# mic-rud/Learned-Compression-of-Point-Cloud-Geometry-and-Attributes

Hardware: AMD Instinct MI355X
Metric: encode+decode Mpoints/sec (higher is better)
Workload: dtype f32

## Files before the change

### include/pcc_hip.h

```cpp
#ifndef PCC_HIP_H
#define PCC_HIP_H

#include <stdint.h>

#ifdef __cplusplus
extern "C" {
#endif

#define PCC_OK 0
#define PCC_ERR_ARG (-1)
#define PCC_ERR_HIP (-2)
#define PCC_ERR_UNSUPPORTED (-3)
#define PCC_ERR_DATA (-4)

#define PCC_ACT_NONE 0
#define PCC_ACT_RELU 1
#define PCC_ACT_LEAKY_RELU 2

int pcc_version(void);
const char* pcc_last_error(void);
int pcc_device_count(void);
int pcc_device_name(int dev, char* out, int out_len);

int64_t pcc_hash_capacity(int64_t n);
// ... 30 lines not shown
int pcc_voxelize(const float* xyz, const int32_t* batch, int64_t n, int32_t nbatch, const float* attr, int32_t c,
                 float origin_x, float origin_y, float origin_z, float voxel, int32_t rounding, uint64_t* keys,
                 int32_t* vals, int64_t cap, int32_t* scratch, int32_t* out_coords, int32_t* out_first,
                 int32_t* out_npts, int64_t* out_sum, int32_t* out_row, int64_t* out_count, void* stream);

int pcc_kernel_map(const int32_t* out_coords, int64_t n_out, const uint64_t* in_keys,
                   const int32_t* in_vals, int64_t in_cap, int32_t ksize, int32_t step,
                   int32_t sign, int32_t* nbr, uint32_t* row_mask, int64_t* pair_count,
                   void* stream);

int pcc_pair_count(const uint32_t* row_mask, int64_t n_out, int64_t* pair_count, void* stream);

int64_t pcc_order_scratch_bytes(int64_t n);
int pcc_order_rows_by_mask(const uint32_t* row_mask, const int32_t* coords, int64_t n,
                           int32_t block_log2, int32_t tensor_stride, int32_t* order, uint32_t* group_mask32,
                           void* scratch, int64_t scratch_bytes, void* stream);
int pcc_permute_map_rows(const int32_t* nbr, const int32_t* order, int64_t n, int32_t K, int32_t* nbr_sorted, void* stream);

int64_t pcc_small_map_max(void);
int32_t pcc_small_paths(int32_t mask);
int pcc_small_kernel_map(const int32_t* out_coords, int64_t n_out, const uint64_t* in_keys, const int32_t* in_vals, int64_t in_cap,
                         int32_t ksize, int32_t step, int32_t sign, int32_t* nbr, uint32_t* row_mask, int32_t* order,
                         uint32_t* group_mask32, void* scratch, int64_t scratch_bytes, void* stream);

int64_t pcc_conv_packed_elems(int32_t K, int32_t cin, int32_t cout);
int pcc_conv_pack_weights(const float* w, int32_t K, int32_t cin, int32_t cout, float* w_packed,
                          void* stream);
int pcc_conv_fwd(const float* fin, int64_t n_in, int32_t cin, const float* w, const float* w_packed,
                 const float* bias, const int32_t* nbr, const int32_t* order,
                 const uint32_t* group_mask32, int32_t K, float* fout, int64_t n_out, int32_t cout,
                 int32_t act, const float* film, const float* residual, void* stream);

int64_t pcc_conv_small_max(int64_t workgroups);

int pcc_conv_kernel_name(int32_t mode, int64_t n_in, int32_t cin, int32_t cout, int64_t n_out, int32_t K, int32_t has_nbr,
                         char* buf, int32_t len);

int64_t pcc_conv_packed_elems_bf16(int32_t K, int32_t cin, int32_t cout);
int pcc_conv_pack_weights_bf16(const float* w, int32_t K, int32_t cin, int32_t cout, uint16_t* w_packed, void* stream);
int pcc_conv_fwd_bf16(const uint16_t* fin, int64_t n_in, int32_t cin, const uint16_t* w_packed, const float* bias,
                      const int32_t* nbr, const int32_t* order, const uint32_t* group_mask32, int32_t K, float* fout,
                      int64_t n_out, int32_t cout, int32_t act, const float* film, const float* residual, void* stream);

int pcc_epilogue_fwd(const float* c, const float* film, const float* residual, int64_t n, int32_t channels, int32_t act,
                     float* out, void* stream);
int pcc_epilogue_bwd(const float* dout, const float* c, const float* film, int64_t n, int32_t channels, int32_t act,
                     float* dc, float* dfilm, void* stream);

int64_t pcc_cast_colsum_scratch_elems(int32_t channels);
int pcc_cast_colsum(const float* x, int64_t n, int32_t channels, uint16_t* out_bf16, float* colsum, float* scratch,
                    int64_t scratch_elems, void* stream);

int64_t pcc_conv_packed_elems_x3(int32_t K, int32_t cin, int32_t cout);
int pcc_conv_pack_weights_x3(const float* w, int32_t K, int32_t cin, int32_t cout, uint16_t* w_packed, void* stream);
int pcc_conv_fwd_x3(const float* fin, int64_t n_in, int32_t cin, const uint16_t* w_packed, const float* bias,
                    const int32_t* nbr, const int32_t* order, const uint32_t* group_mask32, int32_t K, float* fout,
                    int64_t n_out, int32_t cout, int32_t act, const float* film, const float* residual, void* stream);

int pcc_im2col_thin(const float* fin, int32_t cin, const int32_t* nbr, int64_t n_out, int32_t K, float* out, int32_t k2,
                    void* stream);

int pcc_gather_sum_fwd(const float* scores, int32_t ld, const int32_t* nbr, int32_t K, int32_t cout,
                       const float* bias, float* out, int64_t n_out, int32_t act, void* stream);

int pcc_gather_rows(const float* src, int32_t c, const int32_t* idx, int64_t n, float* out,
                    int32_t accumulate, void* stream);
// ... 126 lines not shown
```

### learned-compression-of-point-cloud-geometry-and-attributes_amd/_build.py

```python
import os
import subprocess

_HERE = os.path.dirname(os.path.abspath(__file__))
SO_PATH = os.path.join(_HERE, "libpcc_hip.so")

NO_SCRATCH = {
    "conv": ("conv_small_kernel", "conv_mfma_buf_kernel", "conv_mfma_kernel"),
    "rans_lanes": ("rans_lanes_encode_kernel", "rans_lanes_pack_kernel", "rans_lanes_decode_kernel"),
    "chconv": ("chconv_kernel",),
    "augment": ("jitter_partial_kernel", "jitter_mean_kernel", "jitter_apply_kernel", "first_rows_clear_kernel",
                "first_rows_insert_kernel", "first_rows_flag_kernel", "first_rows_finalize_kernel"),
    "normals": ("estimate_normals_kernel",),
    "voxelize": ("first_rows_clear_kernel", "first_rows_insert_kernel", "first_rows_flag_kernel", "first_rows_finalize_kernel",
                 "voxelize_accumulate_kernel"),
    "raht": ("raht_plan_kernel", "raht_step_kernel", "raht_fold_kernel"),
}


def build(force=False):
    args = ["make", "-s", "-C", os.path.join(_HERE, "csrc"), "-j4"]
    if force:
        subprocess.check_call(args + ["clean"])
    subprocess.check_call(args)
    for stem, kernels in NO_SCRATCH.items():
        check_kernel_resources(os.path.join(_HERE, "build", stem + ".resources.txt"), kernels)
    check_small_kernel_lds_reads()
    return SO_PATH


def check_small_kernel_lds_reads(obj=None):
    import glob
    import shutil
    objdump = "/opt/rocm/lib/llvm/bin/llvm-objdump"
    obj = obj or os.path.join(_HERE, "build", "conv.o")
    if not os.path.exists(objdump) or not os.path.exists(obj):
        raise RuntimeError(f"cannot lint conv_small_kernel: {objdump} or {obj} is missing")
    tmp = os.path.join(_HERE, "build", "_lint")
    shutil.rmtree(tmp, ignore_errors=True)
    os.makedirs(tmp)
    local = os.path.join(tmp, "conv.o")
# ... 84 lines not shown
```

### learned-compression-of-point-cloud-geometry-and-attributes_amd/csrc/conv.hip

```cpp
#include <stdlib.h>

#include <type_traits>

#include "common.h"

namespace pcc {

typedef float f32x2 __attribute__((ext_vector_type(2)));
typedef float f32x4 __attribute__((ext_vector_type(4)));
typedef __bf16 bf16x8 __attribute__((ext_vector_type(8)));

struct ConvArgs {
    const float* fin;
    const float* w;
    const float* wp;
    const float* bias;
    const int32_t* nbr;
    const int32_t* order;
    const uint32_t* gmask;
    float* fout;
    const float* film;
    const float* residual;
    int64_t n_in, n_out;
    int cin, cout, coutp, K, act;
// ... 172 lines not shown
__device__ __forceinline__ unsigned live_tiles(const uint32_t (&mmask)[MT], int k) {
    unsigned live = 0;
#pragma unroll
    for (int m = 0; m < MT; ++m) live |= ((mmask[m] >> k) & 1u) << m;
    return live;
}

template <int MT, class F>
__device__ __forceinline__ void for_live_pattern(unsigned live, F&& block) {
    if constexpr (MT == 1) {
        if (live) block(std::integral_constant<unsigned, 1u>{});
    } else {
        static_assert(MT == 2, "live-pattern dispatch written for MT <= 2");
        if (live == 3u) block(std::integral_constant<unsigned, 3u>{});
        else if (live == 1u) block(std::integral_constant<unsigned, 1u>{});
        else if (live == 2u) block(std::integral_constant<unsigned, 2u>{});
    }
}

template <int MT, int NT>
__device__ __forceinline__ void conv_store_tiles(const ConvArgs& a, const f32x16 (&acc)[MT][NT], int64_t pos0, int col0, int h) {
#pragma unroll
    for (int m = 0; m < MT; ++m) {
#pragma unroll
        for (int n = 0; n < NT; ++n) {
            const int col = col0 + 32 * n;
            if (col >= a.cout) continue;
            const float bcol = conv_bias(a, col);
#pragma unroll
            for (int reg = 0; reg < 16; ++reg) {
                const int64_t pos = pos0 + 32 * m + 4 * h + mfma32_row(reg);
                if (pos >= a.n_out) continue;
                conv_store(a, a.order ? a.order[pos] : pos, col, acc[m][n][reg], bcol);
            }
        }
    }
}

template <int BM, int BN, int WAVES_M, int WAVES_N, bool HAS_NBR>
__global__ __launch_bounds__(256) void conv_mfma_kernel(const ConvArgs a) {
    constexpr int RPT = BM / 32;
    constexpr int WM = BM / WAVES_M, WN = BN / WAVES_N;
    constexpr int MT = WM / 32, NT = WN / 32;
    constexpr int A_LD = A_LD_DMA;
    constexpr int A_ELEMS = BM * A_LD;
    constexpr int W_ELEMS = 8 * BN * 4;
    constexpr int W_LOADS = (8 * BN) / 256;
    static_assert(WAVES_M * WAVES_N == 4 && MT >= 1 && NT >= 1 && W_LOADS >= 1, "bad tiling");

    extern __shared__ __attribute__((aligned(16))) float smem[];
    float* As = smem;
    float* Ws = smem + 2 * A_ELEMS;

    const int t = threadIdx.x;
    const int lane = t & 63, wid = t >> 6;
    const int r = lane & 31, h = lane >> 5;
    const int wrow = (wid / WAVES_N) * WM, wcol = (wid % WAVES_N) * WN;

    const int ntiles_n = a.coutp / BN;
    const int64_t tile = blockIdx.x / ntiles_n;
    const int nt = blockIdx.x - (int)(tile * ntiles_n);
    const int64_t row0 = tile * BM;
    const int CCH = a.cin / 32;
    const int K = a.K;

    uint32_t mmask[MT];
// ... 310 lines not shown
                if constexpr (c + 1 < CCH) {
                    dma(k, std::integral_constant<int, c + 1>{}, std::integral_constant<int, buf ^ 1>{});
                } else {
                    set_src(knext >= 0);
                    dma(knext >= 0 ? knext : k, std::integral_constant<int, 0>{}, std::integral_constant<int, buf ^ 1>{});
                    load_idx(kn2);
                }
                compute(std::integral_constant<int, buf>{}, live);
                __syncthreads();
            });
            const bool more = knext >= 0;
            k = more ? knext : k;
            rem = rem2;
            return more;
        };

        load_idx(k);
        set_src(true);
        dma(k, std::integral_constant<int, 0>{}, std::integral_constant<int, 0>{});
        load_idx(rem ? __builtin_ctz(rem) : k);
        __syncthreads();
        while (true) {
            if (!offset_body(std::integral_constant<int, 0>{})) break;
            if constexpr (CCH & 1) {
                if (!offset_body(std::integral_constant<int, 1>{})) break;
            }
        }
    }

    conv_store_tiles(a, acc, row0 + wrow, nt * BN + wcol + r, h);
#endif
}

template <int SC, int NS>
constexpr int conv_small_lds_bytes() { return (NS * SC * (32 * 32 + 8 * 32 * 4) + 32 * 32) * (int)sizeof(float); }

template <int SC, int NS>
__global__ __launch_bounds__(512) void conv_small_kernel(const ConvArgs a) {
#if defined(__HIP_DEVICE_COMPILE__)
    constexpr int A_STAGE = SC * 32 * 32;
    constexpr int W_STAGE = SC * 8 * 32 * 4;
    constexpr int STAGE = A_STAGE + W_STAGE;
    constexpr int DMAS = 2 * SC;
    static_assert(NS >= 2 && (NS - 1) * DMAS <= 63, "vmcnt is a 6-bit counter");
    extern __shared__ __attribute__((aligned(16))) float smem[];
    int* idx_s = reinterpret_cast<int*>(smem + NS * STAGE);

    const int t = threadIdx.x;
    const int lane = t & 63;
    const int wave_u = __builtin_amdgcn_readfirstlane(t >> 6);
    const int K = a.K;
    const int ntiles_n = a.coutp / 32;
    const int64_t tile = blockIdx.x / ntiles_n;
    const int nt = blockIdx.x - (int)(tile * ntiles_n);
    const int64_t row0 = tile * 32;
    uint32_t tmask = (K >= 32) ? 0xffffffffu : ((1u << K) - 1u);
    if (a.gmask) tmask &= a.gmask[row0 >> 5];
    tmask = __builtin_amdgcn_readfirstlane(tmask);
    const int CG = (a.cin / 32) / SC;
    const int total = __builtin_popcount(tmask) * CG;
    constexpr int WAIT_FIRST = (NS - 1) * DMAS, WAIT_LOOP = (NS - 2) * DMAS;

    if (tmask != 0u) {
        for (int e = t; e < 32 * K; e += 512) {
            const int lr = e / K;
            const int64_t pos = row0 + lr;
// ... 237 lines not shown
            for (int64_t u = w; u < words; ++u) idx_s[u] = src[u];
        }
    }
    __syncthreads();
    if ((int64_t)threadIdx.x >= rows) return;
    const int32_t* mine = idx_s + threadIdx.x * 27;
    float acc[COUT];
#pragma unroll
    for (int c = 0; c < COUT; ++c) acc[c] = 0.0f;
#pragma unroll
    for (int k0 = 0; k0 < 27; k0 += 9) {
        int idx[9];
        float v[9][COUT];
#pragma unroll
        for (int u = 0; u < 9; ++u) idx[u] = mine[k0 + u];
#pragma unroll
        for (int u = 0; u < 9; ++u) {
            const float* sp = scores + (int64_t)(idx[u] >= 0 ? idx[u] : 0) * ld + (k0 + u) * COUT;
#pragma unroll
            for (int c = 0; c < COUT; ++c) v[u][c] = sp[c];
        }
#pragma unroll
        for (int u = 0; u < 9; ++u)
            if (idx[u] >= 0) {
#pragma unroll
                for (int c = 0; c < COUT; ++c) acc[c] += v[u][c];
            }
    }
    float* o = out + (row0 + threadIdx.x) * COUT;
#pragma unroll
    for (int c = 0; c < COUT; ++c) o[c] = apply_act(acc[c] + (bias ? bias[c] : 0.0f), act);
}

enum ConvMode { CONV_F32 = 0, CONV_BF16 = 1, CONV_X3 = 2 };
static const char* const CONV_ENTRY[] = {"pcc_conv_fwd", "pcc_conv_fwd_bf16", "pcc_conv_fwd_x3"};
static const char* const CONV_TAG[] = {"", "[bf16]", "[x3]"};

enum ConvFamily { FAM_THIN, FAM_SMALL, FAM_BUF, FAM_GLOBAL };

struct ConvPlan {
    ConvFamily family;
    int bm, bn, wm, wn;
    int cch;
    int sc, ns;
    int cpt;
};

constexpr int64_t FILL_WGS = 768;
constexpr int64_t ROW32_MAX_WGS = 3000;

static inline int round_up32(int v) { return (v + 31) / 32 * 32; }

static bool fits_buffer_path(const ConvArgs& a) {
    const uint64_t lim = BUF_OOB;
    return (uint64_t)a.n_in * a.cin * 4 <= lim && (uint64_t)a.n_out * a.K * 4 <= lim && (uint64_t)a.K * a.cin * a.coutp * 4 <= lim;
}

static int conv_path() {
    static int path = -1;
    if (path < 0) { const char* e = getenv("PCC_CONV_PATH"); path = (e && e[0] == 'g') ? 1 : 0; }
    return path;
}

static int64_t g_small_max = -1;
static int64_t small_max_value() {
    if (g_small_max < 0) { const char* e = getenv("PCC_CONV_SMALL_MAX"); g_small_max = e ? atoll(e) : 640; }
    return g_small_max;
}

static bool thin_cin(int cin) {
    for (int c : {1, 2, 3, 4, 6, 8, 12, 16, 24})
        if (cin == c) return true;
    return false;
}

static int check_shape(const ConvArgs& a, ConvMode mode, const char* who) {
    PCC_REQUIRE(a.K >= 1 && a.K <= 27, "%s: K=%d out of range", who, a.K);
    if (mode == CONV_F32) PCC_REQUIRE(a.cin % 32 != 0 || a.cin <= 256, "%s: MFMA path supports cin <= 256 (got %d)", who, a.cin);
    if (mode == CONV_BF16) PCC_REQUIRE(a.cin % 64 == 0 && a.cin <= 256, "%s: cin must be a multiple of 64 up to 256 (got %d)", who, a.cin);
    if (mode == CONV_X3) PCC_REQUIRE(a.cin % 32 == 0 && a.cin <= 256, "%s: cin must be a multiple of 32 up to 256 (got %d)", who, a.cin);
    PCC_REQUIRE(a.nbr != nullptr || (a.K == 1 && a.n_in == a.n_out), "%s: nbr == NULL needs K == 1 and n_in == n_out", who);
    return PCC_OK;
}

static int plan_conv(const ConvArgs& a, ConvMode mode, ConvPlan& p, const char* who) {
    p = ConvPlan{};
    if (mode == CONV_F32 && a.cin % 32 != 0) {
        if (!thin_cin(a.cin)) {
            pcc::set_error("%s: unsupported cin=%d (need a multiple of 32 or one of 1,2,3,4,6,8,12,16,24)", who, a.cin);
            return PCC_ERR_UNSUPPORTED;
        }
        const size_t lds = (size_t)a.K * a.cin * a.cout * sizeof(float);
        PCC_REQUIRE(lds <= 160 * 1024, "conv(thin): weights %zu B exceed the 160 KB of LDS (cin=%d cout=%d K=%d)", lds, a.cin, a.cout, a.K);
        p.family = FAM_THIN;
        p.cpt = (a.cout % 8 == 0) ? 8 : (a.cout % 4 == 0) ? 4 : (a.cout % 2 == 0) ? 2 : 1;
        return PCC_OK;
    }
    const bool wide = a.coutp % 128 == 0;
    p.family = FAM_BUF;
    p.cch = a.cin / (mode == CONV_BF16 ? 64 : 32);
    if (mode == CONV_F32) {
        const bool buffer = conv_path() == 0 && fits_buffer_path(a);
        const int64_t wgs32 = ((a.n_out + 31) / 32) * (a.coutp / 32);
        if (a.nbr && buffer && wgs32 <= small_max_value() * (wide ? 1 : 2)) {
            p.family = FAM_SMALL;
            p.sc = (p.cch % 4 == 0 && wgs32 <= 256) ? 4 : p.cch % 2 == 0 ? 2 : 1;
            p.ns = p.sc == 1 ? 8 : 3;
            return PCC_OK;
        }
        if (!buffer) p.family = FAM_GLOBAL;
    } else if (mode == CONV_BF16) {
        PCC_REQUIRE((uint64_t)a.n_in * a.cin * 2 <= BUF_OOB && (uint64_t)a.n_out * a.K * 4 <= BUF_OOB,
                    "%s: operands of 4 GiB and more are not supported", who);
    } else {
        PCC_REQUIRE((uint64_t)a.n_in * a.cin * 4 <= BUF_OOB && (uint64_t)a.n_out * a.K * 4 <= BUF_OOB &&
                    (uint64_t)a.K * a.cin * a.coutp * 6 <= BUF_OOB, "%s: operands of 4 GiB and more are not supported", who);
    }
    const int64_t wgs128 = ((a.n_out + 63) / 64) * (a.coutp / 128);
    auto tile = [&](int bm, int bn, int wm, int wn) { p.bm = bm; p.bn = bn; p.wm = wm; p.wn = wn; return PCC_OK; };
    if (wide && wgs128 < FILL_WGS) return tile(64, 64, 2, 2);
    if (wide && mode == CONV_F32 && wgs128 < ROW32_MAX_WGS) return tile(32, 128, 1, 4);
    if (wide) return tile(64, 128, 2, 2);
    if (a.coutp % 64 == 0) return mode == CONV_X3 ? tile(64, 64, 2, 2) : tile(128, 64, 2, 2);
    if (mode != CONV_X3) return tile(128, 32, 4, 1);
    pcc::set_error("%s: cout=%d not supported (output width rounded up to 32 must be a multiple of 64)", who, a.cout);
    return PCC_ERR_UNSUPPORTED;
}

template <auto KERN>
static int launch(int64_t blocks, int threads, size_t lds, size_t lds_limit, const ConvArgs& a, hipStream_t st) {
    static bool limit_set = false;
    if (lds_limit && !limit_set) {
        PCC_CHECK_HIP(hipFuncSetAttribute(reinterpret_cast<const void*>(KERN), hipFuncAttributeMaxDynamicSharedMemorySize, (int)lds_limit));
        limit_set = true;
    }
    PCC_REQUIRE(blocks < (1ll << 31), "conv: grid too large");
    hipLaunchKernelGGL(KERN, dim3((unsigned)blocks), dim3(threads), lds, st, a);
    PCC_LAUNCH_CHECK();
    return PCC_OK;
}

template <ConvMode M, int BM, int BN, int WM, int WN, int CCH>
static int launch_buf(int64_t blocks, const ConvArgs& a, hipStream_t st) {
    constexpr bool BF16 = M == CONV_BF16, X3 = M == CONV_X3;
    if constexpr (BF16 && CCH > 4) {
        return PCC_ERR_UNSUPPORTED;
    } else {
        constexpr int lds = conv_lds_bytes<BM, BN, X3>();
        return a.nbr ? launch<conv_mfma_buf_kernel<BM, BN, WM, WN, CCH, true, BF16, X3>>(blocks, 256, lds, lds, a, st)
                     : launch<conv_mfma_buf_kernel<BM, BN, WM, WN, CCH, false, BF16, X3>>(blocks, 256, lds, lds, a, st);
    }
}

template <ConvMode M, int BM, int BN, int WM, int WN>
// ... 39 lines not shown
}

template <int CIN>
static int launch_thin(const ConvPlan& p, const ConvArgs& a, hipStream_t st) {
    const size_t lds = (size_t)a.K * CIN * a.cout * sizeof(float);
    const unsigned nb = blocks_for(a.n_out * (a.cout / p.cpt), 256, lds >= 4096 ? 2048u : (1u << 20));
    const size_t limit = lds > 64 * 1024 ? 160 * 1024 : 0;
    if (p.cpt == 8) return launch<conv_thin_kernel<CIN, 8>>(nb, 256, lds, limit, a, st);
    if (p.cpt == 4) return launch<conv_thin_kernel<CIN, 4>>(nb, 256, lds, limit, a, st);
    if (p.cpt == 2) return launch<conv_thin_kernel<CIN, 2>>(nb, 256, lds, limit, a, st);
    return launch<conv_thin_kernel<CIN, 1>>(nb, 256, lds, limit, a, st);
}

static int launch_thin_cin(const ConvPlan& p, const ConvArgs& a, hipStream_t st) {
    switch (a.cin) {
        case 1: return launch_thin<1>(p, a, st);
        case 2: return launch_thin<2>(p, a, st);
        case 3: return launch_thin<3>(p, a, st);
        case 4: return launch_thin<4>(p, a, st);
        case 6: return launch_thin<6>(p, a, st);
        case 8: return launch_thin<8>(p, a, st);
        case 12: return launch_thin<12>(p, a, st);
        case 16: return launch_thin<16>(p, a, st);
        case 24: return launch_thin<24>(p, a, st);
        default: return PCC_ERR_UNSUPPORTED;
    }
}

static int conv_fwd(ConvMode mode, const ConvArgs& a, void* stream) {
    const char* who = CONV_ENTRY[mode];
    int rc = check_shape(a, mode, who);
    if (rc != PCC_OK) return rc;
    PCC_REQUIRE(a.act >= 0 && a.act <= 2, "%s: bad activation %d", who, a.act);
    if (mode == CONV_F32 && a.n_out <= 0) return PCC_OK;
    if (mode != CONV_F32 || a.cin % 32 == 0) {
        PCC_REQUIRE(a.wp != nullptr, "%s: MFMA path (cin=%d) needs packed weights", who, a.cin);
        PCC_REQUIRE(((reinterpret_cast<uintptr_t>(a.fin) | reinterpret_cast<uintptr_t>(a.wp)) & 15) == 0,
                    "%s: fin and w_packed must be 16-byte aligned (16-byte LDS-DMA loads)", who);
    } else {
        PCC_REQUIRE(a.w != nullptr, "%s: thin path (cin=%d) needs raw weights", who, a.cin);
    }
    if (a.n_out <= 0) return PCC_OK;
    ConvPlan p;
    if ((rc = plan_conv(a, mode, p, who)) != PCC_OK) return rc;
    hipStream_t st = as_stream(stream);
    switch (p.family) {
        case FAM_THIN: return launch_thin_cin(p, a, st);
        case FAM_SMALL:
            if (p.sc == 4) return launch_small<4, 3>(a, st);
            return p.sc == 2 ? launch_small<2, 3>(a, st) : launch_small<1, 8>(a, st);
        default:
            if (mode == CONV_BF16) return launch_tile<CONV_BF16>(p, a, st);
            return mode == CONV_X3 ? launch_tile<CONV_X3>(p, a, st) : launch_tile<CONV_F32>(p, a, st);
    }
}

template <class T>
static int pack_weights(const char* who, void (*kern)(const float*, int, int, int, int, int, T*), int cin_pad, const float* w,
                        int K, int cin, int cout, T* w_packed, void* stream) {
    PCC_REQUIRE(K >= 1 && cin >= 1 && cout >= 1, "%s: bad shape", who);
    const int cinp = (cin + cin_pad - 1) / cin_pad * cin_pad, coutp = round_up32(cout);
    const int64_t total = (int64_t)K * cinp * coutp;
    hipLaunchKernelGGL(kern, dim3(blocks_for(total, 256, 4096)), dim3(256), 0, as_stream(stream), w, K, cin, cout, cinp, coutp,
                       w_packed);
    PCC_LAUNCH_CHECK();
    return PCC_OK;
}

}

using namespace pcc;

extern "C" {

int64_t pcc_conv_packed_elems(int32_t K, int32_t cin, int32_t cout) {
    return (int64_t)K * round_up32(cin) * round_up32(cout);
}

int pcc_conv_pack_weights(const float* w, int32_t K, int32_t cin, int32_t cout, float* w_packed, void* stream) {
    return pack_weights("pcc_conv_pack_weights", pack_weights_kernel, 32, w, K, cin, cout, w_packed, stream);
}

int64_t pcc_conv_packed_elems_bf16(int32_t K, int32_t cin, int32_t cout) {
// ... 44 lines not shown
    PCC_REQUIRE(K >= 1 && K <= 27 && cout >= 1 && ld >= K * cout, "pcc_gather_sum_fwd: bad shape (K=%d cout=%d ld=%d)", K, cout, ld);
    PCC_REQUIRE(nbr != nullptr, "pcc_gather_sum_fwd: neighbour table required");
    PCC_REQUIRE(act >= 0 && act <= 2, "pcc_gather_sum_fwd: bad activation %d", act);
    if (n_out <= 0) return PCC_OK;
    const unsigned nb27 = blocks_for(n_out, 256);
    const bool al16 = (reinterpret_cast<uintptr_t>(nbr) & 15) == 0;
#define PCC_GS27(C)                                                                                                    \
    hipLaunchKernelGGL(gather_sum27_kernel<C>, dim3(nb27), dim3(256), 0, as_stream(stream), scores, ld, nbr, bias, out, n_out, act)
    if (K == 27 && al16 && cout == 1) PCC_GS27(1);
    else if (K == 27 && al16 && cout == 2) PCC_GS27(2);
    else if (K == 27 && al16 && cout == 3) PCC_GS27(3);
    else if (K == 27 && al16 && cout == 4) PCC_GS27(4);
    else
#undef PCC_GS27
        hipLaunchKernelGGL(gather_sum_kernel, dim3(blocks_for(n_out * cout, 256, 1 << 20)), dim3(256), 0, as_stream(stream),
                           scores, ld, nbr, K, cout, bias, out, n_out, act);
    PCC_LAUNCH_CHECK();
    return PCC_OK;
}

int64_t pcc_conv_small_max(int64_t workgroups) {
    const int64_t before = small_max_value();
    if (workgroups >= 0) g_small_max = workgroups;
    return before;
}

int pcc_conv_fwd(const float* fin, int64_t n_in, int32_t cin, const float* w, const float* w_packed, const float* bias,
                 const int32_t* nbr, const int32_t* order, const uint32_t* group_mask32, int32_t K, float* fout,
                 int64_t n_out, int32_t cout, int32_t act, const float* film, const float* residual, void* stream) {
    return conv_fwd(CONV_F32, {fin, w, w_packed, bias, nbr, order, group_mask32, fout, film, residual, n_in, n_out, cin, cout,
                               round_up32(cout), K, act}, stream);
}

int pcc_conv_kernel_name(int32_t mode, int64_t n_in, int32_t cin, int32_t cout, int64_t n_out, int32_t K, int32_t has_nbr,
                         char* buf, int32_t len) {
    PCC_REQUIRE(mode >= CONV_F32 && mode <= CONV_X3, "pcc_conv_kernel_name: bad mode %d", mode);
    static const int32_t any_map = 0;
    ConvArgs a = {};
    a.nbr = has_nbr ? &any_map : nullptr;
    a.n_in = n_in; a.n_out = n_out; a.cin = cin; a.cout = cout; a.coutp = round_up32(cout); a.K = K;
    const ConvMode m = ConvMode(mode);
    ConvPlan p;
    if (check_shape(a, m, CONV_ENTRY[m]) != PCC_OK || plan_conv(a, m, p, CONV_ENTRY[m]) != PCC_OK) return PCC_ERR_UNSUPPORTED;
    if (buf == nullptr) return PCC_OK;
    const char* tf = has_nbr ? "true" : "false";
    int n;
    if (p.family == FAM_THIN) n = snprintf(buf, len, "conv_thin_kernel<%d, %d>", cin, p.cpt);
    else if (p.family == FAM_SMALL) n = snprintf(buf, len, "conv_small_kernel<%d, %d>", p.sc, p.ns);
    else if (p.family == FAM_GLOBAL) n = snprintf(buf, len, "conv_mfma_kernel<%d, %d, %d, %d, %s>", p.bm, p.bn, p.wm, p.wn, tf);
    else n = snprintf(buf, len, "conv_mfma_buf_kernel%s<%d, %d, %d, %d, %d, %s>", CONV_TAG[m], p.bm, p.bn, p.wm, p.wn, p.cch, tf);
    PCC_REQUIRE(n < len, "pcc_conv_kernel_name: %d bytes do not hold the name", len);
    return PCC_OK;
}

}
```

### learned-compression-of-point-cloud-geometry-and-attributes_amd/sparse.py

```python
import ctypes
import functools
import math
import weakref

import os

import torch
import torch.nn as nn

from . import _lib, _threads
from ._lib import PCC, check, ptr

ACT_NONE, ACT_RELU, ACT_LRELU = PCC.ACT_NONE, PCC.ACT_RELU, PCC.ACT_LEAKY_RELU


def _require_cuda(t):
    if not t.is_cuda:
        raise RuntimeError("libpcc_hip operators need tensors on an MI355X device (got a CPU tensor); "
                           "there is no CPU fallback")


COORD_PROFILER = None


# ... 480 lines not shown
    n = logits.shape[0]
    dev = logits.device
    ks = [int(v) for v in k_per_batch]
    assert len(ks) == nbatch, (len(ks), nbatch)
    if nbatch == 1:
        k = torch.full((1,), ks[0], dtype=torch.int32, device=dev)
    else:
        k = torch.tensor(ks, dtype=torch.int32).pin_memory().to(dev, non_blocking=True)
    state = torch.empty(L.pcc_topk_state_elems(nbatch), dtype=torch.int32, device=dev)
    mask = torch.empty(n, dtype=torch.uint8, device=dev)
    ev = _cp_begin()
    check(L.pcc_topk_mask(ptr(logits), logits.stride(0), ptr(coords), n, nbatch, ptr(k), ptr(mask), ptr(state),
                          _lib.stream()))
    _cp_end(ev, "top_k", n, 37 * n)
    return mask


def conv_forward(x_feats, in_map, out_map, layer, ksize, transposed=False, act=ACT_NONE, film=None,
                 residual=None, out_channels=None):
    L = _lib.lib()
    w, wp, bias = layer.weights(out_channels)
    n_in, cin = x_feats.shape
    cout = w.shape[-1]
    if ksize > 1 and cin % 32 == 0 and cout <= NARROW_HEAD_MAX_COUT and film is None and residual is None:
        return _narrow_head_forward(x_feats, in_map, out_map, layer, ksize, transposed, act, out_channels)
    if (ksize > 1 and cin in (1, 2, 4, 8) and cout % 32 == 0 and ksize ** 3 * cin <= 256
            and out_map.n * ((ksize ** 3 * cin + 31) // 32 * 32) * 4 < 0xFFFFF000):
        return _thin_im2col_forward(x_feats, in_map, out_map, layer, ksize, transposed, act, film, residual, out_channels)
    nbr, order, gmask, pairs = in_map.conv_map(out_map, ksize, transposed, cin)
    K = ksize ** 3
    n_out = out_map.n
    out = torch.empty((n_out, cout), dtype=torch.float32, device=x_feats.device)
    mode = launch_mode(INFER_BF16, INFER_X3, n_in, cin, cout, n_out, K, nbr is not None) if INFER_BF16 or INFER_X3 else MODE_F32
    prof = PROFILER
    timed = prof is not None and n_out >= PROFILER_MIN_ROWS
    if not timed and mode == MODE_F32:
        check(L.pcc_conv_fwd(x_feats.data_ptr(), n_in, cin, w.data_ptr(), None if wp is None else wp.data_ptr(),
                             None if bias is None else bias.data_ptr(), None if nbr is None else nbr.data_ptr(),
                             None if order is None else order.data_ptr(), None if gmask is None else gmask.data_ptr(), K,
                             out.data_ptr(), n_out, cout, act, None if film is None else film.data_ptr(),
                             None if residual is None else residual.data_ptr(), _lib.stream()))
        if prof is not None:
            prof.append((("conv", mode, n_in, K, nbr is not None), cin, cout, pairs if pairs is not None else n_out, n_out,
                         None, None, gmask))
        return out
    ev0 = _prof_begin(timed)
    launch_conv(mode, x_feats, w, layer.packed(mode, out_channels), bias, nbr, order, gmask, out, act, film, residual)
    _prof_end(ev0, ("conv", mode, n_in, K, nbr is not None), cin, cout, pairs if pairs is not None else n_out, n_out, gmask)
    return out


def profiled_name(entry):
    name, cin, cout, _, n_out = entry[:5]
    if isinstance(name, tuple):
        _, mode, n_in, K, has_nbr = name
        return conv_kernel_name(mode, n_in, cin, cout, n_out, K, has_nbr)
    return name


def _prof_begin(timed=True):
    if PROFILER is None or not timed:
        return None
    ev = torch.cuda.Event(enable_timing=True)
    ev.record()
    return ev


def _prof_end(ev0, name, cin, cout, pairs, n_out, gmask=None):
    if PROFILER is None:
        return
# ... 46 lines not shown

def set_conv_small_max(workgroups):
    return int(_lib.lib().pcc_conv_small_max(int(workgroups)))


NARROW_HEAD_MAX_COUT = 4

CHECK_EXPECTED_COUNTS = os.environ.get("PCC_CHECK_COUNTS", "0") == "1"
ORDER_BLOCK_LOG2 = int(os.environ.get("PCC_ORDER_BLOCK_LOG2", "-1"))

INFER_BF16 = os.environ.get("PCC_INFER_BF16", "0") == "1"


def set_infer_bf16(enabled):
    global INFER_BF16
    INFER_BF16 = bool(enabled)


INFER_X3 = os.environ.get("PCC_INFER_X3", "0") == "1"


def set_infer_x3(enabled):
    global INFER_X3
    INFER_X3 = bool(enabled)


GATE_LOG = None


PROFILER = None
PROFILER_MIN_ROWS = 65536


MODE_F32, MODE_BF16, MODE_X3 = 0, 1, 2


def conv_kernel_name(mode, n_in, cin, cout, n_out, K, has_nbr):
    buf = ctypes.create_string_buffer(128)
    check(_lib.lib().pcc_conv_kernel_name(mode, n_in, cin, cout, n_out, K, int(has_nbr), buf, len(buf)))
    return buf.value.decode()


def launch_mode(bf16, x3, n_in, cin, cout, n_out, K, has_nbr):
    if bf16 and _plan_takes(MODE_BF16, n_in, cin, cout, n_out, K, has_nbr):
        return MODE_BF16
    if x3 and _plan_takes(MODE_X3, n_in, cin, cout, n_out, K, has_nbr):
        return MODE_X3
    return MODE_F32


@functools.lru_cache(maxsize=4096)
def _plan_takes(mode, n_in, cin, cout, n_out, K, has_nbr):
    return _lib.lib().pcc_conv_kernel_name(mode, n_in, cin, cout, n_out, K, int(has_nbr), None, 0) == 0


def launch_conv(mode, feats, w, wp, bias, nbr, order, gmask, out, act=ACT_NONE, film=None, residual=None):
    L = _lib.lib()
    K, cin, cout = w.shape
    n_in, n_out = feats.shape[0], out.shape[0]
    if mode == MODE_BF16:
        check(L.pcc_conv_fwd_bf16(ptr(feats.to(torch.bfloat16)), n_in, cin, ptr(wp), ptr(bias), ptr(nbr), ptr(order), ptr(gmask), K,
                                  ptr(out), n_out, cout, act, ptr(film), ptr(residual), _lib.stream()))
    elif mode == MODE_X3:
        check(L.pcc_conv_fwd_x3(ptr(feats), n_in, cin, ptr(wp), ptr(bias), ptr(nbr), ptr(order), ptr(gmask), K, ptr(out), n_out,
                                cout, act, ptr(film), ptr(residual), _lib.stream()))
    else:
        check(L.pcc_conv_fwd(ptr(feats), n_in, cin, ptr(w), ptr(wp), ptr(bias), ptr(nbr), ptr(order), ptr(gmask), K, ptr(out),
                             n_out, cout, act, ptr(film), ptr(residual), _lib.stream()))


def pack_weights(w, mode=MODE_F32):
    K, cin, cout = w.shape
    if mode == MODE_F32 and cin % 32:
        return None
    L = _lib.lib()
    suffix = ("", "_bf16", "_x3")[mode]
    wp = torch.empty(getattr(L, "pcc_conv_packed_elems" + suffix)(K, cin, cout),
                     dtype=torch.float32 if mode == MODE_F32 else torch.bfloat16, device=w.device)
    check(getattr(L, "pcc_conv_pack_weights" + suffix)(ptr(w), K, cin, cout, ptr(wp), _lib.stream()))
    return wp


def _cached_weights(slot, with_bias=True):
    def wrap(f):
        @functools.wraps(f)
        def cached(self, out_channels=None):
            params = self._parameters
            kernel, bias = params["kernel"], params.get("bias") if with_bias else None
            key = (kernel._version, kernel.data_ptr(), out_channels, None if bias is None else (bias._version, bias.data_ptr()))
            hit = self._packed.get(slot)
            if hit is not None and hit[0] == key:
                return hit[1]
            res = f(self, out_channels)
            self._packed[slot] = (key, res)
            return res
        return cached
    return wrap


class _ConvBase(nn.Module):
    transposed = False
# ... 191 lines not shown
```

Before: 8.927.

## Add persistent run kernel chaining row tiles for transposed sparse convs

Adds conv_mfma_run_kernel, where each workgroup walks a run of four consecutive 64-row tiles. While the current tile finishes its MFMA steps, it prefetches the next tile's group masks, order indices and neighbor indices and starts its first LDS-DMA, so the pipeline does not drain between tiles. A new 'short' conv mode, selected for transposed convs with a neighbor map, forces 64x64 tiling and uses the run kernel when cin is 128 and the grid is large. The cost is a more complex prefetch schedule and fewer workgroups, which lowers parallelism.

```diff
diff --git a/include/pcc_hip.h b/include/pcc_hip.h
--- a/include/pcc_hip.h
+++ b/include/pcc_hip.h
@@ -86,6 +86,12 @@
                  int32_t act, const float* film, const float* residual, void* stream);
 
 int64_t pcc_conv_small_max(int64_t workgroups);
+
+int pcc_conv_fwd_short(const float* fin, int64_t n_in, int32_t cin, const float* w, const float* w_packed,
+                       const float* bias, const int32_t* nbr, const int32_t* order,
+                       const uint32_t* group_mask32, int32_t K, float* fout, int64_t n_out, int32_t cout,
+                       int32_t act, const float* film, const float* residual, void* stream);
+int32_t pcc_conv_short_chain(int32_t variant);
 
 int pcc_conv_kernel_name(int32_t mode, int64_t n_in, int32_t cin, int32_t cout, int64_t n_out, int32_t K, int32_t has_nbr,
                          char* buf, int32_t len);
diff --git a/learned-compression-of-point-cloud-geometry-and-attributes_amd/_build.py b/learned-compression-of-point-cloud-geometry-and-attributes_amd/_build.py
--- a/learned-compression-of-point-cloud-geometry-and-attributes_amd/_build.py
+++ b/learned-compression-of-point-cloud-geometry-and-attributes_amd/_build.py
@@ -5,7 +5,7 @@
 SO_PATH = os.path.join(_HERE, "libpcc_hip.so")
 
 NO_SCRATCH = {
-    "conv": ("conv_small_kernel", "conv_mfma_buf_kernel", "conv_mfma_kernel"),
+    "conv": ("conv_small_kernel", "conv_mfma_buf_kernel", "conv_mfma_kernel", "conv_mfma_run_kernel"),
     "rans_lanes": ("rans_lanes_encode_kernel", "rans_lanes_pack_kernel", "rans_lanes_decode_kernel"),
     "chconv": ("chconv_kernel",),
     "augment": ("jitter_partial_kernel", "jitter_mean_kernel", "jitter_apply_kernel", "first_rows_clear_kernel",
diff --git a/learned-compression-of-point-cloud-geometry-and-attributes_amd/csrc/conv.hip b/learned-compression-of-point-cloud-geometry-and-attributes_amd/csrc/conv.hip
--- a/learned-compression-of-point-cloud-geometry-and-attributes_amd/csrc/conv.hip
+++ b/learned-compression-of-point-cloud-geometry-and-attributes_amd/csrc/conv.hip
@@ -228,6 +228,30 @@
                 const int64_t pos = pos0 + 32 * m + 4 * h + mfma32_row(reg);
                 if (pos >= a.n_out) continue;
                 conv_store(a, a.order ? a.order[pos] : pos, col, acc[m][n][reg], bcol);
+            }
+        }
+    }
+}
+
+template <int MT, int NT>
+__device__ __forceinline__ void conv_store_tiles_rows_first(const ConvArgs& a, const f32x16 (&acc)[MT][NT], int64_t pos0, int col0, int h) {
+#pragma unroll
+    for (int m = 0; m < MT; ++m) {
+        int row[16];
+#pragma unroll
+        for (int reg = 0; reg < 16; ++reg) {
+            const int64_t pos = pos0 + 32 * m + 4 * h + mfma32_row(reg);
+            row[reg] = a.order[pos < a.n_out ? pos : a.n_out - 1];
+        }
+#pragma unroll
+        for (int n = 0; n < NT; ++n) {
+            const int col = col0 + 32 * n;
+            if (col >= a.cout) continue;
+            const float bcol = conv_bias(a, col);
+#pragma unroll
+            for (int reg = 0; reg < 16; ++reg) {
+                if (pos0 + 32 * m + 4 * h + mfma32_row(reg) >= a.n_out) continue;
+                conv_store(a, row[reg], col, acc[m][n][reg], bcol);
             }
         }
     }
@@ -604,6 +628,207 @@
 #endif
 }
 
+template <int BM, int BN, int WAVES_M, int WAVES_N, int CCH, int R>
+__global__ __launch_bounds__(256) void conv_mfma_run_kernel(const ConvArgs a) {
+#if defined(__HIP_DEVICE_COMPILE__)
+    constexpr int RPT = BM / 32, G = BM / 32;
+    constexpr int WM = BM / WAVES_M, WN = BN / WAVES_N;
+    constexpr int MT = WM / 32, NT = WN / 32;
+    constexpr int A_ELEMS = BM * 32;
+    constexpr int W_ELEMS = 8 * BN * 4;
+    constexpr int W_LOADS = (8 * BN) / 256;
+    static_assert(WAVES_M * WAVES_N == 4 && MT >= 1 && MT <= 2 && NT >= 1 && W_LOADS >= 1, "bad tiling");
+    static_assert(CCH >= 4 && CCH % 2 == 0 && R >= 1, "the prefetch schedule needs steps 0, 1 and a last one, on buffer parity 0");
+
+    extern __shared__ __attribute__((aligned(16))) float smem[];
+    float* As = smem;
+    float* Ws = smem + 2 * A_ELEMS;
+
+    const int t = threadIdx.x;
+    const int lane = t & 63, wid = t >> 6;
+    const int r = lane & 31, h = lane >> 5;
+    const int wrow = (wid / WAVES_N) * WM, wcol = (wid % WAVES_N) * WN;
+
+    const int ntiles_n = a.coutp / BN;
+    const int64_t run = blockIdx.x / ntiles_n;
+    const int nt = blockIdx.x - (int)(run * ntiles_n);
+    const int64_t tiles = (a.n_out + BM - 1) / BM;
+    const int n_run = (int)((tiles - run * R < R) ? tiles - run * R : R);
+    const int K = a.K;
+    const uint32_t all = (K >= 32) ? 0xffffffffu : ((1u << K) - 1u);
+    const int64_t ng = (a.n_out + 31) >> 5;
+
+    __amdgpu_buffer_rsrc_t rsrc_a = __builtin_amdgcn_make_buffer_rsrc(const_cast<float*>(a.fin), 0, (int)(uint32_t)(a.n_in * a.cin * 4), BUF_FLAGS);
+    __amdgpu_buffer_rsrc_t rsrc_w = __builtin_amdgcn_make_buffer_rsrc(const_cast<float*>(a.wp), 0, (int)((uint32_t)K * a.cin * a.coutp * 4), BUF_FLAGS);
+    __amdgpu_buffer_rsrc_t rsrc_n = __builtin_amdgcn_make_buffer_rsrc(const_cast<int32_t*>(a.nbr), 0, (int)(uint32_t)(a.n_out * K * 4), BUF_FLAGS);
+
+    const int gchunk = t & 7;
+    int grow[RPT];
+    uint32_t q16[RPT], a_voff[RPT];
+#pragma unroll
+    for (int i = 0; i < RPT; ++i) {
+        grow[i] = wid * (BM / 4) + 8 * i + (lane >> 3);
+        q16[i] = (uint32_t)((gchunk ^ ((grow[i] >> 1) & 7)) * 16);
+    }
+    uint32_t w_voff[W_LOADS];
+#pragma unroll
+    for (int j = 0; j < W_LOADS; ++j) {
+        const int f = t + 256 * j;
+        const int g = f / BN, col = f - g * BN;
+        w_voff[j] = (uint32_t)((g * a.coutp + nt * BN + col) * 16);
+    }
+    const int wave_u = __builtin_amdgcn_readfirstlane(wid);
+    const uint32_t w_kstride = (uint32_t)(a.cin / 4) * a.coutp * 16;
+    const uint32_t w_cstride = 8u * a.coutp * 16;
+    const uint32_t a_row_bytes = (uint32_t)a.cin * 4;
+    uint32_t a_addr[2][4], w_addr[2];
+#pragma unroll
+    for (int b = 0; b < 2; ++b) {
+#pragma unroll
+        for (int kk = 0; kk < 4; ++kk) a_addr[b][kk] = (uint32_t)(b * A_ELEMS * 4) + a_frag_offset(wrow + r, h, kk);
+        w_addr[b] = (uint32_t)((2 * A_ELEMS + b * W_ELEMS + (h * BN + wcol + r) * 4) * 4);
+    }
+    auto dma = [&](int k, int c, int buf) __attribute__((always_inline)) {
+#pragma unroll
+        for (int i = 0; i < RPT; ++i)
+            __builtin_amdgcn_raw_ptr_buffer_load_lds(rsrc_a, (lds_ptr_t)(As + buf * A_ELEMS + (wave_u * RPT + i) * 256), 16, a_voff[i], c * 128, 0, 0);
+        const uint32_t wso = (uint32_t)k * w_kstride + (uint32_t)c * w_cstride;
+#pragma unroll
+        for (int j = 0; j < W_LOADS; ++j)
+            __builtin_amdgcn_raw_ptr_buffer_load_lds(rsrc_w, (lds_ptr_t)(Ws + buf * W_ELEMS + (wave_u * 64 + 256 * j) * 4), 16, w_voff[j], wso, 0, 0);
+    };
+
+    uint32_t raw_gm[G];
+    int raw_ord[RPT];
+    auto fetch = [&](int64_t row0n) __attribute__((always_inline)) {
+        const int64_t g0 = row0n >> 5;
+#pragma unroll
+        for (int g = 0; g < G; ++g) {
+            const int64_t gi = g0 + g < ng ? g0 + g : ng - 1;
+            raw_gm[g] = a.gmask[gi];
+        }
+#pragma unroll
+        for (int i = 0; i < RPT; ++i) {
+            const int64_t pos = row0n + grow[i];
+            const int64_t ps = pos < a.n_out ? pos : a.n_out - 1;
+            raw_ord[i] = a.order[ps];
+        }
+    };
+    auto resolve = [&](int64_t row0n, uint32_t& tm, uint32_t (&mm)[MT], uint32_t (&voff)[RPT], bool (&valid)[RPT]) __attribute__((always_inline)) {
+        uint32_t any = 0u;
+#pragma unroll
+        for (int g = 0; g < G; ++g) any |= raw_gm[g];
+        tm = __builtin_amdgcn_readfirstlane(any) & all;
+#pragma unroll
+        for (int m = 0; m < MT; ++m) {
+            uint32_t v = 0u;
+#pragma unroll
+            for (int g = 0; g < G; ++g) v = (g == (wrow >> 5) + m) ? raw_gm[g] : v;
+            mm[m] = __builtin_amdgcn_readfirstlane(v) & all;
+        }
+#pragma unroll
+        for (int i = 0; i < RPT; ++i) {
+            valid[i] = row0n + grow[i] < a.n_out;
+            voff[i] = (uint32_t)((int64_t)raw_ord[i] * K * 4);
+        }
+    };
+
+    int64_t row0 = run * R * BM;
+    uint32_t tmask, mmask[MT], n_voff[RPT];
+    bool rvalid[RPT];
+    int idx_nxt[RPT];
+    fetch(row0);
+    resolve(row0, tmask, mmask, n_voff, rvalid);
+    bool primed = false;
+
+    for (int it = 0; it < n_run; ++it) {
+        const bool has_next = it + 1 < n_run;
+        const int64_t row0n = has_next ? row0 + BM : row0;
+        uint32_t nx_tmask = 0u, nx_mmask[MT], nx_voff[RPT];
+        bool nx_rvalid[RPT], nx_live = false;
+        int nx_idx[RPT], nx_k0 = 0, nx_k1 = 0;
+        fetch(row0n);
+        auto resolve_next = [&]() __attribute__((always_inline)) {
+#pragma unroll
+            for (int g = 0; g < G; ++g) asm volatile("" : "+v"(raw_gm[g]));
+            resolve(row0n, nx_tmask, nx_mmask, nx_voff, nx_rvalid);
+            nx_tmask = has_next ? nx_tmask : 0u;
+            nx_live = nx_tmask != 0u;
+            nx_k0 = nx_live ? __builtin_ctz(nx_tmask) : 0;
+            const uint32_t r2 = nx_tmask & (nx_tmask - 1u);
+            nx_k1 = r2 ? __builtin_ctz(r2) : nx_k0;
+        };
+        auto load_idx = [&](const uint32_t (&voff)[RPT], int k, int (&idx)[RPT]) __attribute__((always_inline)) {
+#pragma unroll
+            for (int i = 0; i < RPT; ++i) idx[i] = (int)__builtin_amdgcn_raw_buffer_load_b32(rsrc_n, voff[i], k * 4, 0);
+        };
+
+        f32x16 acc[MT][NT] = {};
+        if (tmask != 0u) {
+            uint32_t rem = tmask;
+            int k = __builtin_ctz(rem);
+            rem &= rem - 1u;
+            if (!primed) {
+                load_idx(n_voff, k, idx_nxt);
+#pragma unroll
+                for (int i = 0; i < RPT; ++i)
+                    a_voff[i] = (rvalid[i] && idx_nxt[i] >= 0) ? (uint32_t)idx_nxt[i] * a_row_bytes + q16[i] : BUF_OOB;
+                dma(k, 0, 0);
+                load_idx(n_voff, rem ? __builtin_ctz(rem) : k, idx_nxt);
+                __syncthreads();
+            }
+            bool more = true;
+            while (more) {
+                const int knext = rem ? __builtin_ctz(rem) : -1;
+                const uint32_t rem2 = rem & (rem - 1u);
+                const int kn2 = rem2 ? __builtin_ctz(rem2) : (knext >= 0 ? knext : k);
+                const unsigned live = live_tiles(mmask, k);
+                more = knext >= 0;
+#pragma unroll
+                for (int c = 0; c < CCH; ++c) {
+                    const int buf = c & 1;
+                    if (c == 1) {
+                        resolve_next();
+                        load_idx(nx_voff, nx_k0, nx_idx);
+                    }
+                    if (c + 1 < CCH) {
+                        dma(k, c + 1, buf ^ 1);
+                    } else {
+#pragma unroll
+                        for (int i = 0; i < RPT; ++i) {
+                            const int idx = more ? idx_nxt[i] : nx_idx[i];
+                            const bool ok = (more ? rvalid[i] : (nx_live && nx_rvalid[i])) && idx >= 0;
+                            a_voff[i] = ok ? (uint32_t)idx * a_row_bytes + q16[i] : BUF_OOB;
+                        }
+                        dma(more ? knext : (nx_live ? nx_k0 : k), 0, buf ^ 1);
+                        const int kload = more ? kn2 : nx_k1;
+#pragma unroll
+                        for (int i = 0; i < RPT; ++i)
+                            idx_nxt[i] = (int)__builtin_amdgcn_raw_buffer_load_b32(rsrc_n, more ? n_voff[i] : nx_voff[i], kload * 4, 0);
+                    }
+                    for_live_pattern<MT>(live, [&](auto live_tag) __attribute__((always_inline)) {
+                        mfma_step<decltype(live_tag)::value, BN, false>(acc, a_addr[buf], w_addr[buf]);
+                    });
+                    __syncthreads();
+                }
+                k = more ? knext : k;
+                rem = rem2;
+            }
+        }
+        conv_store_tiles_rows_first(a, acc, row0 + wrow, nt * BN + wcol + r, h);
+
+        resolve_next();
+        primed = tmask != 0u && nx_live;
+        row0 = row0n;
+        tmask = nx_tmask;
+#pragma unroll
+        for (int m = 0; m < MT; ++m) mmask[m] = nx_mmask[m];
+#pragma unroll
+        for (int i = 0; i < RPT; ++i) { n_voff[i] = nx_voff[i]; rvalid[i] = nx_rvalid[i]; }
+    }
+#endif
+}
+
 template <int SC, int NS>
 constexpr int conv_small_lds_bytes() { return (NS * SC * (32 * 32 + 8 * 32 * 4) + 32 * 32) * (int)sizeof(float); }
 
@@ -907,11 +1132,14 @@
     for (int c = 0; c < COUT; ++c) o[c] = apply_act(acc[c] + (bias ? bias[c] : 0.0f), act);
 }
 
-enum ConvMode { CONV_F32 = 0, CONV_BF16 = 1, CONV_X3 = 2 };
-static const char* const CONV_ENTRY[] = {"pcc_conv_fwd", "pcc_conv_fwd_bf16", "pcc_conv_fwd_x3"};
-static const char* const CONV_TAG[] = {"", "[bf16]", "[x3]"};
-
-enum ConvFamily { FAM_THIN, FAM_SMALL, FAM_BUF, FAM_GLOBAL };
+enum ConvMode { CONV_F32 = 0, CONV_BF16 = 1, CONV_X3 = 2, CONV_SHORT = 3 };
+static const char* const CONV_ENTRY[] = {"pcc_conv_fwd", "pcc_conv_fwd_bf16", "pcc_conv_fwd_x3", "pcc_conv_fwd_short"};
+static const char* const CONV_TAG[] = {"", "[bf16]", "[x3]", ""};
+static inline bool is_f32(ConvMode m) { return m == CONV_F32 || m == CONV_SHORT; }
+
+enum ConvFamily { FAM_THIN, FAM_SMALL, FAM_BUF, FAM_GLOBAL, FAM_RUN };
+constexpr int RUN_TILES = 4;
+constexpr int64_t RUN_MIN_WGS = 8192;
 
 struct ConvPlan {
     ConvFamily family;
@@ -943,6 +1171,12 @@
     return g_small_max;
 }
 
+static int g_short_chain = -1;
+static int short_chain_value() {
+    if (g_short_chain < 0) { const char* e = getenv("PCC_CONV_SHORT_CHAIN"); g_short_chain = e ? atoi(e) : 1; }
+    return g_short_chain;
+}
+
 static bool thin_cin(int cin) {
     for (int c : {1, 2, 3, 4, 6, 8, 12, 16, 24})
         if (cin == c) return true;
@@ -951,7 +1185,7 @@
 
 static int check_shape(const ConvArgs& a, ConvMode mode, const char* who) {
     PCC_REQUIRE(a.K >= 1 && a.K <= 27, "%s: K=%d out of range", who, a.K);
-    if (mode == CONV_F32) PCC_REQUIRE(a.cin % 32 != 0 || a.cin <= 256, "%s: MFMA path supports cin <= 256 (got %d)", who, a.cin);
+    if (is_f32(mode)) PCC_REQUIRE(a.cin % 32 != 0 || a.cin <= 256, "%s: MFMA path supports cin <= 256 (got %d)", who, a.cin);
     if (mode == CONV_BF16) PCC_REQUIRE(a.cin % 64 == 0 && a.cin <= 256, "%s: cin must be a multiple of 64 up to 256 (got %d)", who, a.cin);
     if (mode == CONV_X3) PCC_REQUIRE(a.cin % 32 == 0 && a.cin <= 256, "%s: cin must be a multiple of 32 up to 256 (got %d)", who, a.cin);
     PCC_REQUIRE(a.nbr != nullptr || (a.K == 1 && a.n_in == a.n_out), "%s: nbr == NULL needs K == 1 and n_in == n_out", who);
@@ -960,7 +1194,7 @@
 
 static int plan_conv(const ConvArgs& a, ConvMode mode, ConvPlan& p, const char* who) {
     p = ConvPlan{};
-    if (mode == CONV_F32 && a.cin % 32 != 0) {
+    if (is_f32(mode) && a.cin % 32 != 0) {
         if (!thin_cin(a.cin)) {
             pcc::set_error("%s: unsupported cin=%d (need a multiple of 32 or one of 1,2,3,4,6,8,12,16,24)", who, a.cin);
             return PCC_ERR_UNSUPPORTED;
@@ -974,7 +1208,7 @@
     const bool wide = a.coutp % 128 == 0;
     p.family = FAM_BUF;
     p.cch = a.cin / (mode == CONV_BF16 ? 64 : 32);
-    if (mode == CONV_F32) {
+    if (is_f32(mode)) {
         const bool buffer = conv_path() == 0 && fits_buffer_path(a);
         const int64_t wgs32 = ((a.n_out + 31) / 32) * (a.coutp / 32);
         if (a.nbr && buffer && wgs32 <= small_max_value() * (wide ? 1 : 2)) {
@@ -993,8 +1227,14 @@
     }
     const int64_t wgs128 = ((a.n_out + 63) / 64) * (a.coutp / 128);
     auto tile = [&](int bm, int bn, int wm, int wn) { p.bm = bm; p.bn = bn; p.wm = wm; p.wn = wn; return PCC_OK; };
+    if (mode == CONV_SHORT && p.family == FAM_BUF && short_chain_value() != 0 && a.coutp % 64 == 0) {
+        const int64_t run_wgs = (((a.n_out + 63) / 64 + RUN_TILES - 1) / RUN_TILES) * (a.coutp / 64);
+        const int v = short_chain_value();
+        if (v != 2 && (v == 3 || run_wgs >= RUN_MIN_WGS) && a.nbr && a.order && a.gmask && p.cch == 4) p.family = FAM_RUN;
+        return tile(64, 64, 2, 2);
+    }
     if (wide && wgs128 < FILL_WGS) return tile(64, 64, 2, 2);
-    if (wide && mode == CONV_F32 && wgs128 < ROW32_MAX_WGS) return tile(32, 128, 1, 4);
+    if (wide && is_f32(mode) && wgs128 < ROW32_MAX_WGS) return tile(32, 128, 1, 4);
     if (wide) return tile(64, 128, 2, 2);
     if (a.coutp % 64 == 0) return mode == CONV_X3 ? tile(64, 64, 2, 2) : tile(128, 64, 2, 2);
     if (mode != CONV_X3) return tile(128, 32, 4, 1);
@@ -1100,8 +1340,8 @@
     int rc = check_shape(a, mode, who);
     if (rc != PCC_OK) return rc;
     PCC_REQUIRE(a.act >= 0 && a.act <= 2, "%s: bad activation %d", who, a.act);
-    if (mode == CONV_F32 && a.n_out <= 0) return PCC_OK;
-    if (mode != CONV_F32 || a.cin % 32 == 0) {
+    if (is_f32(mode) && a.n_out <= 0) return PCC_OK;
+    if (!is_f32(mode) || a.cin % 32 == 0) {
         PCC_REQUIRE(a.wp != nullptr, "%s: MFMA path (cin=%d) needs packed weights", who, a.cin);
         PCC_REQUIRE(((reinterpret_cast<uintptr_t>(a.fin) | reinterpret_cast<uintptr_t>(a.wp)) & 15) == 0,
                     "%s: fin and w_packed must be 16-byte aligned (16-byte LDS-DMA loads)", who);
@@ -1117,6 +1357,11 @@
         case FAM_SMALL:
             if (p.sc == 4) return launch_small<4, 3>(a, st);
             return p.sc == 2 ? launch_small<2, 3>(a, st) : launch_small<1, 8>(a, st);
+        case FAM_RUN: {
+            constexpr int lds = conv_lds_bytes<64, 64>();
+            const int64_t runs = ((a.n_out + 63) / 64 + RUN_TILES - 1) / RUN_TILES;
+            return launch<conv_mfma_run_kernel<64, 64, 2, 2, 4, RUN_TILES>>(runs * (a.coutp / 64), 256, lds, lds, a, st);
+        }
         default:
             if (mode == CONV_BF16) return launch_tile<CONV_BF16>(p, a, st);
             return mode == CONV_X3 ? launch_tile<CONV_X3>(p, a, st) : launch_tile<CONV_F32>(p, a, st);
@@ -1227,12 +1472,27 @@
                                round_up32(cout), K, act}, stream);
 }
 
+int pcc_conv_fwd_short(const float* fin, int64_t n_in, int32_t cin, const float* w, const float* w_packed, const float* bias,
+                       const int32_t* nbr, const int32_t* order, const uint32_t* group_mask32, int32_t K, float* fout,
+                       int64_t n_out, int32_t cout, int32_t act, const float* film, const float* residual, void* stream) {
+    return conv_fwd(CONV_SHORT, {fin, w, w_packed, bias, nbr, order, group_mask32, fout, film, residual, n_in, n_out, cin, cout,
+                                 round_up32(cout), K, act}, stream);
+}
+
+int32_t pcc_conv_short_chain(int32_t variant) {
+    const int32_t before = short_chain_value();
+    if (variant >= 0) g_short_chain = variant;
+    return before;
+}
+
 int pcc_conv_kernel_name(int32_t mode, int64_t n_in, int32_t cin, int32_t cout, int64_t n_out, int32_t K, int32_t has_nbr,
                          char* buf, int32_t len) {
-    PCC_REQUIRE(mode >= CONV_F32 && mode <= CONV_X3, "pcc_conv_kernel_name: bad mode %d", mode);
+    PCC_REQUIRE(mode >= CONV_F32 && mode <= CONV_SHORT, "pcc_conv_kernel_name: bad mode %d", mode);
     static const int32_t any_map = 0;
     ConvArgs a = {};
     a.nbr = has_nbr ? &any_map : nullptr;
+    a.order = a.nbr;
+    a.gmask = reinterpret_cast<const uint32_t*>(a.nbr);
     a.n_in = n_in; a.n_out = n_out; a.cin = cin; a.cout = cout; a.coutp = round_up32(cout); a.K = K;
     const ConvMode m = ConvMode(mode);
     ConvPlan p;
@@ -1242,6 +1502,7 @@
     int n;
     if (p.family == FAM_THIN) n = snprintf(buf, len, "conv_thin_kernel<%d, %d>", cin, p.cpt);
     else if (p.family == FAM_SMALL) n = snprintf(buf, len, "conv_small_kernel<%d, %d>", p.sc, p.ns);
+    else if (p.family == FAM_RUN) n = snprintf(buf, len, "conv_mfma_run_kernel<%d, %d, %d, %d, %d, %d>", p.bm, p.bn, p.wm, p.wn, p.cch, RUN_TILES);
     else if (p.family == FAM_GLOBAL) n = snprintf(buf, len, "conv_mfma_kernel<%d, %d, %d, %d, %s>", p.bm, p.bn, p.wm, p.wn, tf);
     else n = snprintf(buf, len, "conv_mfma_buf_kernel%s<%d, %d, %d, %d, %d, %s>", CONV_TAG[m], p.bm, p.bn, p.wm, p.wn, p.cch, tf);
     PCC_REQUIRE(n < len, "pcc_conv_kernel_name: %d bytes do not hold the name", len);
diff --git a/learned-compression-of-point-cloud-geometry-and-attributes_amd/sparse.py b/learned-compression-of-point-cloud-geometry-and-attributes_amd/sparse.py
--- a/learned-compression-of-point-cloud-geometry-and-attributes_amd/sparse.py
+++ b/learned-compression-of-point-cloud-geometry-and-attributes_amd/sparse.py
@@ -536,10 +536,12 @@
     n_out = out_map.n
     out = torch.empty((n_out, cout), dtype=torch.float32, device=x_feats.device)
     mode = launch_mode(INFER_BF16, INFER_X3, n_in, cin, cout, n_out, K, nbr is not None) if INFER_BF16 or INFER_X3 else MODE_F32
+    if mode == MODE_F32 and transposed and nbr is not None:
+        mode = MODE_SHORT
     prof = PROFILER
     timed = prof is not None and n_out >= PROFILER_MIN_ROWS
-    if not timed and mode == MODE_F32:
-        check(L.pcc_conv_fwd(x_feats.data_ptr(), n_in, cin, w.data_ptr(), None if wp is None else wp.data_ptr(),
+    if not timed and mode in (MODE_F32, MODE_SHORT):
+        check((L.pcc_conv_fwd if mode == MODE_F32 else L.pcc_conv_fwd_short)(x_feats.data_ptr(), n_in, cin, w.data_ptr(), None if wp is None else wp.data_ptr(),
                              None if bias is None else bias.data_ptr(), None if nbr is None else nbr.data_ptr(),
                              None if order is None else order.data_ptr(), None if gmask is None else gmask.data_ptr(), K,
                              out.data_ptr(), n_out, cout, act, None if film is None else film.data_ptr(),
@@ -652,7 +654,7 @@
 PROFILER_MIN_ROWS = 65536
 
 
-MODE_F32, MODE_BF16, MODE_X3 = 0, 1, 2
+MODE_F32, MODE_BF16, MODE_X3, MODE_SHORT = 0, 1, 2, 3
 
 
 def conv_kernel_name(mode, n_in, cin, cout, n_out, K, has_nbr):
@@ -685,8 +687,9 @@
         check(L.pcc_conv_fwd_x3(ptr(feats), n_in, cin, ptr(wp), ptr(bias), ptr(nbr), ptr(order), ptr(gmask), K, ptr(out), n_out,
                                 cout, act, ptr(film), ptr(residual), _lib.stream()))
     else:
-        check(L.pcc_conv_fwd(ptr(feats), n_in, cin, ptr(w), ptr(wp), ptr(bias), ptr(nbr), ptr(order), ptr(gmask), K, ptr(out),
-                             n_out, cout, act, ptr(film), ptr(residual), _lib.stream()))
+        fwd = L.pcc_conv_fwd_short if mode == MODE_SHORT else L.pcc_conv_fwd
+        check(fwd(ptr(feats), n_in, cin, ptr(w), ptr(wp), ptr(bias), ptr(nbr), ptr(order), ptr(gmask), K, ptr(out),
+                  n_out, cout, act, ptr(film), ptr(residual), _lib.stream()))
 
 
 def pack_weights(w, mode=MODE_F32):
```

Result: no change. 8.940 (median of 4 runs) (+0.1%).
